# xmindflow/TransCeption

Hardware: AMD Instinct MI355X
Metric: images/sec fwd+bwd at 224x224 B=16 per GPU (higher is better)
Workload: dtype bf16; 1 GPU; TransCeption (MSTransception) 224x224 B=16/GPU fwd+bwd+SGD, synthetic Synapse npz slices via the device loader, name-seeded random-init weights; global_batch=16, image_size=224, parallelism=dp1, headline_mode=loader, headline_degraded=False, launch_mode=hipGraph replay

## Files before the change

transception_amd/_header.py:

```python
from __future__ import annotations

import ctypes as C
import operator
import os
import re
from typing import NamedTuple

HEADER = os.path.join(os.path.dirname(os.path.dirname(os.path.abspath(__file__))), "include", "transception_hip.h")


class SideHeader(NamedTuple):
    attr: str
    file: str
    version: str
    entry: str
    what: str

    @property
    def path(self) -> str:
        return os.path.join(os.path.dirname(HEADER), self.file)


SIDE_HEADERS = (SideHeader("POST", "transception_post.h", "TC_POST_ABI_VERSION", "tc_post_abi_version", "post-processing"),
                SideHeader("EMA", "transception_ema.h", "TC_EMA_ABI_VERSION", "tc_ema_abi_version", "weight-averaging"),
                SideHeader("TTA", "transception_tta.h", "TC_TTA_ABI_VERSION", "tc_tta_abi_version", "test-time augmentation"),
                SideHeader("RESAMPLE", "transception_resample.h", "TC_RESAMPLE_ABI_VERSION", "tc_resample_abi_version", "score resampling"),
                SideHeader("BRIDGE", "transception_bridge.h", "TC_BRIDGE_ABI_VERSION", "tc_bridge_abi_version", "bridge LayerNorm"),
                SideHeader("LOSS", "transception_loss.h", "TC_LOSS_ABI_VERSION", "tc_loss_abi_version", "focal / Tversky loss"))

SCALARS = {"int": C.c_int, "long long": C.c_longlong, "float": C.c_float, "double": C.c_double,
           "unsigned": C.c_uint, "unsigned int": C.c_uint}
POINTEES = set(SCALARS) | {"void", "unsigned char"}


class HeaderError(ValueError):
    pass


class Function(NamedTuple):
    restype: type
    argtypes: list
    query: bool


class Header(NamedTuple):
    functions: dict
    structs: dict
    constants: dict


_TOKEN = re.compile(r"\s*(\d+|<<|[()|+-])")
_LEVELS = ({"|": operator.or_}, {"<<": operator.lshift}, {"+": operator.add, "-": operator.sub})


def evaluate(expr: str) -> int:
    toks, pos, expr = [], 0, expr.strip()
    while pos < len(expr):
        m = _TOKEN.match(expr, pos)
        if not m:
            raise HeaderError(f"constant expression {expr!r}: cannot read {expr[pos:]!r}")
        toks.append(m.group(1))
        pos = m.end()
    toks.reverse()

    def level(i):
        if i == len(_LEVELS):
            t = toks.pop() if toks else ""
            if t in ("-", "+"):
                return level(i) if t == "+" else -level(i)
            if t == "(":
                v = level(0)
                if not toks or toks.pop() != ")":
                    raise HeaderError(f"constant expression {expr!r}: missing )")
                return v
            if t.isdigit():
                return int(t)
            raise HeaderError(f"constant expression {expr!r}: operand expected")
        v = level(i + 1)
        while toks and toks[-1] in _LEVELS[i]:
            v = _LEVELS[i][toks.pop()](v, level(i + 1))
# ... 102 lines not shown
```

transception_amd/_lib.py:

```python
from __future__ import annotations

import ctypes as C
import os

from . import _header

HERE = os.path.dirname(os.path.abspath(__file__))
LIB_PATH = os.environ.get("TC_LIB_PATH") or os.path.join(HERE, "libtransception_hip.so")

ABI = _header.load()
SIGNATURES = {name: f.argtypes for name, f in ABI.functions.items()}
K, S = ABI.constants, ABI.structs
SIDE = {s.attr: _header.load(s.path) for s in _header.SIDE_HEADERS}
POST, EMA, TTA, RESAMPLE, BRIDGE, LOSS = SIDE["POST"], SIDE["EMA"], SIDE["TTA"], SIDE["RESAMPLE"], SIDE["BRIDGE"], SIDE["LOSS"]

ABI_VERSION = K["TC_ABI_VERSION"]
TC_F32, TC_BF16, TC_F16 = K["TC_F32"], K["TC_BF16"], K["TC_F16"]
ACT_NONE, ACT_HSWISH, ACT_COORD, ACT_SIGMOID = K["TC_ACT_NONE"], K["TC_ACT_HSWISH"], K["TC_ACT_COORD"], K["TC_ACT_SIGMOID"]
ACT_GELU, ACT_SCALE, ACT_RELU = K["TC_ACT_GELU"], K["TC_ACT_SCALE"], K["TC_ACT_RELU"]
FFN_NONE, FFN_LN_A, FFN_LN_B, FFN_EP = K["TC_FFN_NONE"], K["TC_FFN_LN_A"], K["TC_FFN_LN_B"], K["TC_FFN_EP"]
EW_PATCHIFY, EW_DEINTERLEAVE, EW_COPY, EW_MULTI_MAX = K["TC_EW_PATCHIFY"], K["TC_EW_DEINTERLEAVE"], K["TC_EW_COPY"], K["TC_EW_MULTI_MAX"]
TC_AUG_WARP, TC_AUG_LINEAR, TC_AUG_BLUR, TC_AUG_PIECEWISE = K["TC_AUG_WARP"], K["TC_AUG_LINEAR"], K["TC_AUG_BLUR"], K["TC_AUG_PIECEWISE"]
TC_AUG_SKIP, TC_AUG_FROM_RAW = K["TC_AUG_SKIP"], K["TC_AUG_FROM_RAW"]
ATTN_DKV_SPLITS = K["TC_ATTN_DKV_SPLITS"]
TC_METRIC_NO_SOURCE, TC_METRIC_SELECT_WORK_BYTES = K["TC_METRIC_NO_SOURCE"], K["TC_METRIC_SELECT_WORK_BYTES"]
TC_IGNORE_NONE = K["TC_IGNORE_NONE"]
POST_ABI_VERSION, EMA_ABI_VERSION, TTA_ABI_VERSION, RESAMPLE_ABI_VERSION, BRIDGE_ABI_VERSION, LOSS_ABI_VERSION = (SIDE[s.attr].constants[s.version] for s in _header.SIDE_HEADERS)
TC_OVERLAP_DICE, TC_OVERLAP_TVERSKY = LOSS.constants["TC_OVERLAP_DICE"], LOSS.constants["TC_OVERLAP_TVERSKY"]
TC_CC_LARGEST, TC_CC_MIN_VOXELS = POST.constants["TC_CC_LARGEST"], POST.constants["TC_CC_MIN_VOXELS"]
TC_RESAMPLE_MAX_EXTENT = RESAMPLE.constants["TC_RESAMPLE_MAX_EXTENT"]
TC_TTA_FLIP_H, TC_TTA_FLIP_W, TC_TTA_TRANSPOSE = TTA.constants["TC_TTA_FLIP_H"], TTA.constants["TC_TTA_FLIP_W"], TTA.constants["TC_TTA_TRANSPOSE"]

TcGemm, TcLnFold, TcDwFold, TcDwSeg, TcFfnSeg = S["TcGemm"], S["TcLnFold"], S["TcDwFold"], S["TcDwSeg"], S["TcFfnSeg"]
TcFfnFused, TcFfnBwd, TcEffAtt, TcEwSeg, TcSliceAug = S["TcFfnFused"], S["TcFfnBwd"], S["TcEffAtt"], S["TcEwSeg"], S["TcSliceAug"]
TcSrSrc, TcLnSeg = BRIDGE.structs["TcSrSrc"], BRIDGE.structs["TcLnSeg"]
SR_LN_MAX, LN_MULTI_MAX = BRIDGE.constants["TC_SR_LN_MAX"], BRIDGE.constants["TC_LN_MULTI_MAX"]


class TcError(RuntimeError):
    pass


class _Lib:
    calls = 0

    def __init__(self, path: str = LIB_PATH):
        if not os.path.exists(path):
            raise TcError(f"{path} is missing: build it with `python -m transception_amd.build` "
                          "(there is no CPU/PyTorch fallback for the TransCeption hot path)")
        self.path = path
        self.cdll = C.CDLL(path)
        headers = [(ABI, "TC_ABI_VERSION", "tc_abi_version", "ABI"),
                   *((SIDE[s.attr], s.version, s.entry, s.what + " ABI") for s in _header.SIDE_HEADERS)]
        for header, *_ in headers:
            for name, f in header.functions.items():
                fn = getattr(self.cdll, name)
                fn.argtypes = f.argtypes
                fn.restype = f.restype
                setattr(self, name, fn if f.query else self._checked(name, fn))
        for header, version, entry, what in headers:
            v, host = getattr(self.cdll, entry)(), header.constants[version]
            if v != host:
                raise TcError(f"{what} mismatch: library {v}, host {host}")

    @staticmethod
    def _checked(name, fn):
        def call(*a):
            _Lib.calls += 1
            rc = fn(*a)
            if rc != 0:
                raise TcError(f"{name} failed with status {rc}")
        call.__name__ = name
        return call


_lib = None


def lib() -> _Lib:
    global _lib
# ... 4 lines not shown
```

transception_amd/csrc/factoratt.hip:

```cpp
#include "tc_common.h"

namespace {

constexpr int FA_MAXCH = 64;

template <typename T>
__device__ __forceinline__ void fa_load_tile(float* dst, const T* src, int ld, int N, int Ch) {
    constexpr int VEC = TcVec16<T>::N;
    const int nv = Ch / VEC, total = N * nv;
#pragma unroll 4
    for (int i = threadIdx.x; i < total; i += 256) {
        const int n = i / nv, cv = i - n * nv;
        const uint4 r = *reinterpret_cast<const uint4*>(src + (long long)n * ld + cv * VEC);
        tc_unpack16<T>(r, dst + n * Ch + cv * VEC);
    }
}

__device__ __forceinline__ void fa_softmax_cols(float* e, float* cmax, float* cinv, float* red, int N, int Ch) {
    const int tid = threadIdx.x, R = 256 / Ch, c = tid % Ch, r = tid / Ch;
    float m = -INFINITY;
    if (r < R) for (int n = r; n < N; n += R) m = fmaxf(m, e[n * Ch + c]);
    if (r < R) red[r * Ch + c] = m;
    __syncthreads();
    if (tid < Ch) { float v = red[tid]; for (int i = 1; i < R; ++i) v = fmaxf(v, red[i * Ch + tid]); cmax[tid] = v; }
    __syncthreads();
    float s = 0.f;
    if (r < R) {
        const float mc = cmax[c];
        for (int n = r; n < N; n += R) { const float v = __expf(e[n * Ch + c] - mc); e[n * Ch + c] = v; s += v; }
        red[r * Ch + c] = s;
    }
    __syncthreads();
    if (tid < Ch) { float v = 0.f; for (int i = 0; i < R; ++i) v += red[i * Ch + tid]; cinv[tid] = 1.0f / v; }
    __syncthreads();
}

template <typename T>
__device__ __forceinline__ void fa_load_tile_raw(T* dst, const T* src, int ld, int N, int Ch) {
    constexpr int VEC = TcVec16<T>::N;
    const int nv = Ch / VEC, total = N * nv;
#pragma unroll 4
    for (int i = threadIdx.x; i < total; i += 256) {
        const int n = i / nv, cv = i - n * nv;
        *reinterpret_cast<uint4*>(dst + n * Ch + cv * VEC) = *reinterpret_cast<const uint4*>(src + (long long)n * ld + cv * VEC);
    }
}
__device__ __forceinline__ float fa_get(const float* p, int i) { return p[i]; }
__device__ __forceinline__ float fa_get(const bf16_t* p, int i) { return bf2f(p[i]); }
__device__ __forceinline__ float fa_get(const f16_t* p, int i) { return h2f(p[i]); }
__device__ __forceinline__ void fa_get8(const float* p, float* o) {
    const float4 a = *reinterpret_cast<const float4*>(p), b = *reinterpret_cast<const float4*>(p + 4);
    o[0] = a.x; o[1] = a.y; o[2] = a.z; o[3] = a.w; o[4] = b.x; o[5] = b.y; o[6] = b.z; o[7] = b.w;
}
// ... 938 lines not shown
            const T* src = xb + (long long)((ok ? yy : y) * p.W + (ok ? xx : x)) * p.ldx + sub * 8;
#pragma unroll
            for (int v = 0; v < NVL; ++v) {
                raw[ky * 3 + kx][v] = *reinterpret_cast<const uint4*>(src + v * 64);
                if (!ok) raw[ky * 3 + kx][v] = make_uint4(0u, 0u, 0u, 0u);
            }
        }
    __syncthreads();
    float t1v[NVL][8];
    float s1 = 0.f;
#pragma unroll
    for (int v = 0; v < NVL; ++v) {
        const int c0 = v * 64 + sub * 8;
        float acc[8], ctr[8];
        tc_unpack16<T>(raw[4][v], ctr);
#pragma unroll
        for (int u = 0; u < 8; ++u) acc[u] = bs[c0 + u];
#pragma unroll
        for (int tap = 0; tap < 9; ++tap) {
            float xv[8], w8[8];
            tc_unpack16<T>(raw[tap][v], xv);
            fa_get8(wt + tap * C + c0, w8);
#pragma unroll
            for (int u = 0; u < 8; ++u) acc[u] = fmaf(xv[u], w8[u], acc[u]);
        }
#pragma unroll
        for (int u = 0; u < 8; ++u) acc[u] += ctr[u];
        const uint4 pk = tc_pack16<T>(acc);
        if (live) *reinterpret_cast<uint4*>(reinterpret_cast<T*>(p.t1) + (grow + r) * p.ldt + c0) = pk;
        tc_unpack16<T>(pk, t1v[v]);
#pragma unroll
        for (int u = 0; u < 8; ++u) s1 += t1v[v][u];
    }
    const float mean = tc_group_sum<8>(s1) * (1.0f / C);
    float s2 = 0.f;
#pragma unroll
    for (int v = 0; v < NVL; ++v)
#pragma unroll
        for (int u = 0; u < 8; ++u) { const float d = t1v[v][u] - mean; s2 += d * d; }
    const float rstd = rsqrtf(tc_group_sum<8>(s2) * (1.0f / C) + p.eps);
    if (live) {
#pragma unroll
        for (int v = 0; v < NVL; ++v) {
            const int c0 = v * 64 + sub * 8;
            float o[8];
#pragma unroll
            for (int u = 0; u < 8; ++u) o[u] = (t1v[v][u] - mean) * rstd * gm[c0 + u] + bt[c0 + u];
            *reinterpret_cast<uint4*>(reinterpret_cast<T*>(p.xn) + (grow + r) * p.ldn + c0) = tc_pack16<T>(o);
        }
        if (sub == 0) { p.mean[grow + r] = mean; p.rstd[grow + r] = rstd; }
    }
}

static size_t mhca_att_smem_of(int C, int N) {
    return C == 64 ? mhca_att_smem<64>(N) : C == 128 ? mhca_att_smem<128>(N) : C == 320 ? mhca_att_smem<320>(N) : 0;
}
extern "C" int tc_mhca_att_supported(int C, int N, int dtype) {
    if (dtype != TC_BF16 && dtype != TC_F16) return 0;
    const size_t sm = mhca_att_smem_of(C, N);
    return sm > 0 && sm <= 150 * 1024 && N > 0;
}
extern "C" int tc_mhca_att_fwd(const void* xn, int ldx, const void* Wqkv, const void* bqkv, const void* w3, const void* b3, const void* w5,
                               const void* b5, const void* w7, const void* b7, long long gs, void* qkv, int ldq, void* convv, int ldc,
                               void* o, int ldo, float* stats, int groups, int B, int H, int W, int C, float scale, int dtype, void* stream) {
    if (!xn || !Wqkv || !bqkv || !w3 || !b3 || !w5 || !b5 || !w7 || !b7 || !qkv || !convv || !o || !stats || groups <= 0 || B <= 0 || H <= 0 || W <= 0)
        return TC_ERR_ARG;
    if (!tc_mhca_att_supported(C, H * W, dtype)) return TC_ERR_UNSUPPORTED;
    {
        const long long n = (long long)H * W, lmax = ldx > ldq ? (ldx > ldc ? ldx : ldc) : (ldq > ldc ? ldq : ldc);
        if (n * (lmax > ldo ? lmax : ldo) >= (1LL << 31) || lmax >= (1 << 23) || ldo >= (1 << 23)) return TC_ERR_ARG;
    }
    if (ldx % 8 || ldq % 8 || ldc % 8 || ldo % 8 || gs % 8 ||
        (((uintptr_t)xn | (uintptr_t)Wqkv | (uintptr_t)qkv | (uintptr_t)convv | (uintptr_t)o) & 15))
        return TC_ERR_ARG;
    MhcaAttDev p;
    p.xn = xn; p.Wqkv = Wqkv; p.bqkv = bqkv; p.cw[0] = w3; p.cw[1] = w5; p.cw[2] = w7; p.cb[0] = b3; p.cb[1] = b5; p.cb[2] = b7;
    p.qkv = qkv; p.convv = convv; p.o = o; p.stats = stats; p.gs = gs; p.ldx = ldx; p.ldq = ldq; p.ldc = ldc; p.ldo = ldo;
    p.B = B; p.N = H * W; p.H = H; p.W = W; p.scale = scale;
    const int Bt = groups * B;
    hipStream_t s = (hipStream_t)stream;
    if (dtype == TC_BF16) {
        if (C == 64) return mhca_att_launch<bf16_t, 64>(p, Bt, s);
        if (C == 128) return mhca_att_launch<bf16_t, 128>(p, Bt, s);
        return mhca_att_launch<bf16_t, 320>(p, Bt, s);
    }
    if (C == 64) return mhca_att_launch<f16_t, 64>(p, Bt, s);
    if (C == 128) return mhca_att_launch<f16_t, 128>(p, Bt, s);
    return mhca_att_launch<f16_t, 320>(p, Bt, s);
}

static size_t mhca_att_bwd_smem_of(int C, int N) {
    return C == 64 ? mhca_att_bwd_smem<64>(N) : C == 128 ? mhca_att_bwd_smem<128>(N) : C == 320 ? mhca_att_bwd_smem<320>(N) : 0;
}
extern "C" int tc_mhca_att_bwd_supported(int C, int N, int dtype) {
    if (dtype != TC_BF16 && dtype != TC_F16) return 0;
    const size_t sm = mhca_att_bwd_smem_of(C, N);
    return sm > 0 && sm <= 79 * 1024 && N > 0;
}
extern "C" int tc_mhca_att_bwd(const void* qkv, int ldq, const void* convv, int ldc, const void* go, int ldgo, const float* stats, void* dqkv,
                               int ldd, int acc_q, int acc_k, int acc_v, const void* w3, const void* w5, const void* w7, float* dw3, float* db3,
                               float* dw5, float* db5, float* dw7, float* db7, long long gs, int groups, int B, int H, int W, int C, float scale,
                               int dtype, void* stream) {
    if (!qkv || !convv || !go || !stats || !dqkv || !w3 || !w5 || !w7 || !dw3 || !db3 || !dw5 || !db5 || !dw7 || !db7 || groups <= 0 || B <= 0 ||
        H <= 0 || W <= 0)
        return TC_ERR_ARG;
    if (!tc_mhca_att_bwd_supported(C, H * W, dtype)) return TC_ERR_UNSUPPORTED;
    {
        const long long n = (long long)H * W, l1 = ldq > ldc ? ldq : ldc, l2 = ldgo > ldd ? ldgo : ldd, lmax = l1 > l2 ? l1 : l2;
        if (n * lmax >= (1LL << 31) || lmax >= (1 << 23)) return TC_ERR_ARG;
    }
    if (ldq % 8 || ldc % 8 || ldgo % 8 || ldd % 8 || (((uintptr_t)qkv | (uintptr_t)convv | (uintptr_t)go | (uintptr_t)dqkv) & 15)) return TC_ERR_ARG;
    MhcaAttBwdDev p;
    p.qkv = qkv; p.convv = convv; p.go = go; p.cw[0] = w3; p.cw[1] = w5; p.cw[2] = w7; p.stats = stats; p.dqkv = dqkv;
    p.dcw[0] = dw3; p.dcw[1] = dw5; p.dcw[2] = dw7; p.dcb[0] = db3; p.dcb[1] = db5; p.dcb[2] = db7; p.gs = gs;
    p.ldq = ldq; p.ldc = ldc; p.ldgo = ldgo; p.ldd = ldd; p.acc_q = acc_q; p.acc_k = acc_k; p.acc_v = acc_v;
    p.B = B; p.N = H * W; p.H = H; p.W = W; p.scale = scale;
    const int Bt = groups * B;
    hipStream_t s = (hipStream_t)stream;
    if (dtype == TC_BF16) {
        if (C == 64) return mhca_att_bwd_launch<bf16_t, 64>(p, Bt, s);
        if (C == 128) return mhca_att_bwd_launch<bf16_t, 128>(p, Bt, s);
        return mhca_att_bwd_launch<bf16_t, 320>(p, Bt, s);
    }
    if (C == 64) return mhca_att_bwd_launch<f16_t, 64>(p, Bt, s);
    if (C == 128) return mhca_att_bwd_launch<f16_t, 128>(p, Bt, s);
    return mhca_att_bwd_launch<f16_t, 320>(p, Bt, s);
}

extern "C" int tc_dw_ln_supported(int C, int dtype) { return (dtype == TC_BF16 || dtype == TC_F16) && (C == 64 || C == 128 || C == 320); }
extern "C" int tc_dw_ln_fwd(const void* x, int ldx, const void* w, const void* b, long long wstride, const void* gamma, const void* beta,
                            long long gstride, void* t1, int ldt, void* xn, int ldn, float* mean, float* rstd, int groups, int B, int H, int W,
                            int C, float eps, int dtype, void* stream) {
    if (!x || !w || !b || !gamma || !beta || !t1 || !xn || !mean || !rstd || groups <= 0 || B <= 0 || H <= 0 || W <= 0) return TC_ERR_ARG;
    if (!tc_dw_ln_supported(C, dtype)) return TC_ERR_UNSUPPORTED;
    if (ldx % 8 || ldt % 8 || ldn % 8 || (((uintptr_t)x | (uintptr_t)t1 | (uintptr_t)xn) & 15)) return TC_ERR_ARG;
    DwLnDev p;
    p.x = x; p.w = w; p.b = b; p.gamma = gamma; p.beta = beta; p.t1 = t1; p.xn = xn; p.mean = mean; p.rstd = rstd;
    p.wstride = wstride; p.gstride = gstride; p.ldx = ldx; p.ldt = ldt; p.ldn = ldn; p.B = B; p.H = H; p.W = W;
    p.rows_per_group = B * H * W; p.eps = eps;
    const dim3 grid((p.rows_per_group + 31) / 32, groups);
    hipStream_t s = (hipStream_t)stream;
#define DWLN(TT, CC) hipLaunchKernelGGL((dw_ln_fwd_kernel<TT, CC>), grid, dim3(256), 0, s, p)
    if (dtype == TC_BF16) { if (C == 64) DWLN(bf16_t, 64); else if (C == 128) DWLN(bf16_t, 128); else DWLN(bf16_t, 320); }
    else { if (C == 64) DWLN(f16_t, 64); else if (C == 128) DWLN(f16_t, 128); else DWLN(f16_t, 320); }
#undef DWLN
    return tc_launch_status();
}
```

transception_amd/engine.py:

```python
from __future__ import annotations

import ctypes as C
import os
from typing import Callable, Dict, List, Optional, Tuple

import torch

from ._lib import (ATTN_DKV_SPLITS, EW_COPY, EW_DEINTERLEAVE, EW_PATCHIFY, TcEffAtt, TcEwSeg, TcFfnBwd, TcFfnFused, ACT_COORD, ACT_GELU, ACT_HSWISH, ACT_NONE, ACT_SCALE, ACT_SIGMOID, FFN_EP, FFN_LN_A, FFN_LN_B, TC_BF16, TC_F16, TC_F32, TcDwFold, TcDwSeg, TcFfnSeg,
                   TcGemm, TcLnFold, TcLnSeg, TcSrSrc, LN_MULTI_MAX, lib)

TC_DTYPE = {torch.float32: TC_F32, torch.bfloat16: TC_BF16, torch.float16: TC_F16}

PROFILE: Optional[dict] = None


SEG_MARKS = os.environ.get("TC_SEG_MARKS", "")
SEG_LABELS: List[str] = []


def _timed(name: str, flops: float, fn):
    if PROFILE is None:
        fn()
        return
    e0, e1 = torch.cuda.Event(enable_timing=True), torch.cuda.Event(enable_timing=True)
# ... 78 lines not shown
    def is_whole(self) -> bool:
        rt = self.root.data
        return self.region == (0, rt.shape[0], 0, rt.shape[1])

    def apply_path(self, t: torch.Tensor) -> torch.Tensor:
        for k in self.path:
            if k[0] == "c":
                t = t[:, k[1]:k[2]]
            elif k[0] == "r":
                t = t[k[1]:k[2]]
            else:
                t = t.view(k[1], k[2])
        return t


def _overlap(a, b) -> bool:
    return a[0] < b[1] and b[0] < a[1] and a[2] < b[3] and b[2] < a[3]


def _ptr(t: Optional[torch.Tensor]):
    return None if t is None else t.data_ptr()


_WORKSPACES: Dict[Tuple[str, str], torch.Tensor] = {}
WORKSPACE_BYTES = 16384 + 1024 * 16384


def _workspace(device, tag: str = "") -> torch.Tensor:
    key = (str(device), tag)
    ws = _WORKSPACES.get(key)
    if ws is None:
        ws = _WORKSPACES[key] = torch.zeros(WORKSPACE_BYTES * (8 if tag == "many" else 1), dtype=torch.uint8, device=device)
    return ws


_SPLITK_CAP = 128
_SPLITK_BLOCKS = 512
_SPLITK_KMIN = 384
_THR128 = 100000
_FFN_STORE_ACT = os.environ.get("TC_FFN_STORE_ACT", "1") != "0"
_FFN_LN_GEMM_MAXC = int(os.environ.get("TC_FFN_LN_GEMM_MAXC", "64"))
_FFN_TILED = os.environ.get("TC_FFN_TILED", "1") != "0"
_DW_DEFER = os.environ.get("TC_DW_DEFER", "1") != "0"
_LN_DEFER = os.environ.get("TC_LN_DEFER", "1") != "0"
_EFFATT_FUSED = os.environ.get("TC_EFFATT_FUSED", "1") != "0"
_FFN_PRE_LN = os.environ.get("TC_FFN_PRE_LN", "0") != "0"
_SR_LN_FUSED = os.environ.get("TC_SR_LN_FUSED", "1") != "0"
_LN_MULTI = os.environ.get("TC_LN_MULTI", "1") != "0"
_PENDING_RES = os.environ.get("TC_PENDING_RES", "1") != "0"
_LIN_LN_FUSED = os.environ.get("TC_LIN_LN_FUSED", "1") != "0"
_RIPM_FUSED = os.environ.get("TC_RIPM_FUSED", "1") != "0"
_LN_CLS_FUSED = os.environ.get("TC_LN_CLS_FUSED", "1") != "0"
_DW_LN_FUSED = os.environ.get("TC_DW_LN_FUSED", "1") != "0"
_MHCA_ATT_BWD_FUSED = os.environ.get("TC_MHCA_ATT_BWD_FUSED", "1") != "0"
_MHCA_ATT_FUSED = os.environ.get("TC_MHCA_ATT_FUSED", "1") != "0"
_DW_BWD_ONE = os.environ.get("TC_DW_BWD_ONE", "1") != "0"
_FFN_TILED_BWD = os.environ.get("TC_FFN_TILED_BWD", "1") != "0"
_FFN_TILE_BWD = (0, 0)
_FFN_TILE = (0, 0)
_POISON = bool(os.environ.get("TC_DEBUG_POISON"))


def _empty(shape, dtype, device) -> torch.Tensor:
    if _POISON:
        return torch.full(tuple(shape), float("nan"), dtype=dtype, device=device)
    return torch.empty(tuple(shape), dtype=dtype, device=device)


_ZERO_NEED: Dict[Tuple[str, torch.dtype], int] = {}


class _ZeroArena:
    def __init__(self, device, dtype):
        self.key = (str(device), dtype)
        self.device, self.dtype = device, dtype
        self.buf: Optional[torch.Tensor] = None
        self.used = 0
        self.asked = 0

    def zeros_like(self, t: torch.Tensor) -> torch.Tensor:
        n = (t.numel() + 127) // 128 * 128
        self.asked += n
        if self.buf is None:
            need = _ZERO_NEED.get(self.key, 0)
            if need >= n:
                self.buf = torch.zeros(need, dtype=self.dtype, device=self.device)
        if self.buf is not None and self.used + n <= self.buf.numel() and t.is_contiguous():
            out = self.buf[self.used:self.used + t.numel()].view(t.shape)
            self.used += n
            return out
        return torch.zeros_like(t)

    def close(self):
        _ZERO_NEED[self.key] = max(self.asked, 0)


class _Grouped:
    def __init__(self, G, n, pgs):
        self.G, self.n, self.pgs, self.prev = G, n, pgs, None

    def __enter__(self):
        self.prev = (self.G.ngroups, self.G.pgs)
        self.G.ngroups, self.G.pgs = self.n, self.pgs
        return self

    def __exit__(self, *a):
# ... 832 lines not shown
        c = x.cols // max(p * p, 1)
        ncls = Wc.data.shape[0]
        rows = B * H * p * W * p if p else x.rows
        out = self.new(rows, (ncls + 7) // 8 * 8).colslice(0, ncls) if pad_rows else self.new(rows, ncls)
        mean, rstd = self.f32(rows), self.f32(rows)
        es = x.data.element_size()
        self.n_launch += 1
        _timed("hbm:ln_cls_fwd (pixel shuffle + LayerNorm + classifier, one launch)", 1.0 * rows * (c + ncls) * es, lambda: self.L.tc_ln_cls_fwd(
            _ptr(x.data), x.ld, _ptr(g.data), _ptr(b.data), _ptr(Wc.data), _ptr(bc.data), _ptr(out.data), out.ld, _ptr(mean), _ptr(rstd),
            B, H, W, p, c, ncls, eps, self.dt, self.stream))

        def bwd():
            dl = self.grad_of(out)
            if dl is None or not x.requires_grad:
                return
            gx, acc = self.wgrad(x)
            assert not acc, "the expanded map has one consumer"
            n = int(self.L.tc_ln_cls_scratch_floats(rows, ncls))
            scratch = self.f32(n)
            _timed("hbm:ln_cls_bwd", 1.0 * rows * (2 * c + ncls) * es, lambda: self.L.tc_ln_cls_bwd(
                _ptr(dl), dl.stride(0), _ptr(x.data), x.ld, _ptr(g.data), _ptr(b.data), _ptr(Wc.data), _ptr(mean), _ptr(rstd), _ptr(gx), gx.stride(0),
                _ptr(g.grad), _ptr(b.grad), _ptr(Wc.grad), _ptr(bc.grad), _ptr(scratch), n, B, H, W, p, c, ncls, self.dt, self.stream))
        self._rec(bwd)
        return out

    def linear_ln_supported(self, x: Var, W: P, residual: Optional[Var], *params: P) -> bool:
        Cc = x.cols
        return (all(q.data.data_ptr() % 16 == 0 for q in params) and _LIN_LN_FUSED and self.dt != TC_F32 and tuple(W.data.shape) == (Cc, Cc) and W.data.is_contiguous()
                and x.ld % 8 == 0 and x.data.data_ptr() % 16 == 0 and (residual is None or (residual.ld % 8 == 0 and residual.data.data_ptr() % 16 == 0))
                and (self.ngroups == 1 or self.pgs % 8 == 0) and bool(self.L.tc_linear_ln_supported(Cc, self.dt)))

    def linear_ln(self, x: Var, W: P, b: P, residual: Optional[Var], g: P, beta: P, eps: float, out: Optional[Var] = None,
                  ln_out: Optional[Var] = None) -> Tuple[Var, Var]:
        Gn = self.ngroups
        t = self.linear(x, W, b, out=out, residual=residual, launch=False)
        mean, rstd = self.f32(x.rows), self.f32(x.rows)
        xn = self.layernorm(t, g, beta, eps, out=ln_out, stats=(mean, rstd), launch=False)
        assert t.rows == x.rows and t.cols == x.cols, "row-stacked groups only"
        self.n_launch += 1
        es = x.data.element_size()
        _timed("hbm:linear_ln_fwd (Linear + residual + LayerNorm, one launch)", (4.0 if residual is not None else 3.0) * x.rows * x.cols * es,
               lambda: self.L.tc_linear_ln_fwd(_ptr(x.data), x.ld, _ptr(W.data), _ptr(b.data), W.gs if Gn > 1 else 0,
                                               _ptr(residual.data) if residual is not None else None, residual.ld if residual is not None else 0,
                                               _ptr(g.data), _ptr(beta.data), g.gs if Gn > 1 else 0, _ptr(t.data), t.ld, _ptr(xn.data), xn.ld,
                                               _ptr(mean), _ptr(rstd), Gn, x.rows // Gn, x.cols, eps, self.dt, self.stream))
        return t, xn

    def dw_ln_supported(self, x: Var) -> bool:
        return (_DW_LN_FUSED and self.dt != TC_F32 and x.ld % 8 == 0 and x.data.data_ptr() % 16 == 0
                and (self.pgs % 8 == 0 or self.ngroups == 1) and bool(self.L.tc_dw_ln_supported(x.cols, self.dt)))

    def dw_ln(self, x: Var, w: P, b: P, g: P, beta: P, B: int, H: int, W: int, eps: float) -> Tuple[Var, Var]:
        Gn = self.ngroups
        t1 = self.dwconv(x, w, b, B, H, W, 3, 1, True, launch=False)
        mean, rstd = self.f32(x.rows), self.f32(x.rows)
        xn = self.layernorm(t1, g, beta, eps, stats=(mean, rstd), launch=False)
        self.n_launch += 1
        es = x.data.element_size()
        _timed("hbm:dw_ln_fwd (cpe dw3x3 + skip + LayerNorm, one launch)", 3.0 * x.rows * x.cols * es, lambda: self.L.tc_dw_ln_fwd(
            _ptr(x.data), x.ld, _ptr(w.data), _ptr(b.data), w.gs if Gn > 1 else 0, _ptr(g.data), _ptr(beta.data), g.gs if Gn > 1 else 0,
            _ptr(t1.data), t1.ld, _ptr(xn.data), xn.ld, _ptr(mean), _ptr(rstd), Gn, B, H, W, x.cols, eps, self.dt, self.stream))
        return t1, xn

    def dwconv(self, x: Var, w: P, b: Optional[P], B: int, H: int, W: int, k: int, stride: int = 1, add_input: bool = False,
               out: Optional[Var] = None, launch: bool = True) -> Var:
        Cc = x.cols
        Gn = self.ngroups
        assert x.rows == Gn * B * H * W and (Gn == 1 or (w.gs > 0 and stride == 1))
        Ho, Wo = (H - 1) // stride + 1, (W - 1) // stride + 1
        if out is None:
            out = self.new(Gn * B * Ho * Wo, Cc)
        es = x.data.element_size()
        if launch:
            _timed("hbm:dwconv_fwd", (x.rows + out.rows) * Cc * es, lambda: self.L.tc_dwconv_fwd(
                _ptr(x.data), x.ld, _ptr(w.data), _ptr(b.data) if b is not None else None, _ptr(out.data), out.ld, B, H, W, Cc, k, stride,
                int(add_input), Gn, w.gs, self.dt, self.stream))

        def bwd():
            dy = self.grad_of(out)
            if dy is None:
                return
            if x.requires_grad and w.grad is not None and stride == 1 and _DW_BWD_ONE:
                gx, acc = self.wgrad(x)
                vec = 16 // es
                db = _ptr(b.grad) if b is not None else None
                tile_ok = not (x.ld % vec or dy.stride(0) % vec or gx.stride(0) % vec or _ptr(dy) % 16 or _ptr(x.data) % 16 or _ptr(gx) % 16)
                self._dw_walkers(
                    (lambda sites, offs: self.L.tc_dwconv_bwd_plan(B, H, W, Cc, k, Gn, self.dt, C.byref(sites[0]))) if _DW_DEFER and tile_ok else None,
                    lambda wsp, wsb: _timed("hbm:dwconv_bwd (input + weight gradient, one launch)", (2.0 * x.rows * (1 + acc) + 2.0 * out.rows) * Cc * es,
                                            lambda: self.L.tc_dwconv_bwd(_ptr(dy), dy.stride(0), _ptr(x.data), x.ld, _ptr(w.data), _ptr(gx), gx.stride(0),
                                                                         _ptr(w.grad), db, B, H, W, Cc, k, int(add_input), acc, Gn, w.gs, wsp, wsb,
                                                                         self.dt, self.stream)),
                    [(_ptr(w.grad), db, None, None, w.gs)])
                return
            if x.requires_grad:
                gx, acc = self.wgrad(x)
                _timed("hbm:dwconv_bwd_input", (x.rows * (1 + acc) + out.rows) * Cc * es, lambda: self.L.tc_dwconv_bwd_input(
                    _ptr(dy), dy.stride(0), _ptr(w.data), _ptr(gx), gx.stride(0), B, H, W, Cc, k, stride, int(add_input), acc, Gn, w.gs,
                    self.dt, self.stream))
            if w.grad is not None:
                ws = _workspace(self.dev)
                _timed("hbm:dwconv_bwd_weight", (x.rows + out.rows) * Cc * es, lambda: self.L.tc_dwconv_bwd_weight(
                    _ptr(dy), dy.stride(0), _ptr(x.data), x.ld, _ptr(w.grad), _ptr(b.grad) if b is not None else None, B, H, W, Cc, k,
                    stride, Gn, w.gs, ws.data_ptr(), ws.numel(), self.dt, self.stream))
        self._rec(bwd)
        return out

    def dwconv_multi(self, xs: List[Var], ws: List[P], bs: List[Optional[P]], geo, ks: List[int], outs: List[Optional[Var]],
                     add_input: bool = False, launch: bool = True) -> List[Var]:
# ... 856 lines not shown
```

Measured before the change: 1518 images/sec.

## Fuse LayerNorm backward with depthwise 3x3 conv backward in one kernel

After: 1516 images/sec. About the same (-0.1%).

```diff
diff --git a/include/transception_mhca.h b/include/transception_mhca.h
--- /dev/null
+++ b/include/transception_mhca.h
@@ -0,0 +1,24 @@
+#ifndef TRANSCEPTION_MHCA_H
+#define TRANSCEPTION_MHCA_H
+
+#ifdef __cplusplus
+extern "C" {
+#endif
+
+#define TC_MHCA_ABI_VERSION 1
+#ifndef TC_QUERY
+#define TC_QUERY
+#endif
+
+TC_QUERY int tc_mhca_abi_version(void);
+
+TC_QUERY int tc_dw_ln_bwd_walkers(int groups, int B, int H, int W, int C, int dtype);
+int tc_dw_ln_bwd(const void* dxn, int lddn, const void* t1, int ldt, const void* x, int ldx, const void* w, long long wstride,
+                 const void* gamma, long long gstride, const float* mean, const float* rstd, const void* dres, int ldres, void* gx, int ldg,
+                 int acc, float* ln_part, long long ln_part_floats, float* dw_part, long long dw_part_floats, int groups, int B, int H, int W,
+                 int C, int dtype, void* stream);
+
+#ifdef __cplusplus
+}
+#endif
+#endif
diff --git a/transception_amd/_header.py b/transception_amd/_header.py
--- a/transception_amd/_header.py
+++ b/transception_amd/_header.py
@@ -26,6 +26,7 @@
                 SideHeader("TTA", "transception_tta.h", "TC_TTA_ABI_VERSION", "tc_tta_abi_version", "test-time augmentation"),
                 SideHeader("RESAMPLE", "transception_resample.h", "TC_RESAMPLE_ABI_VERSION", "tc_resample_abi_version", "score resampling"),
                 SideHeader("BRIDGE", "transception_bridge.h", "TC_BRIDGE_ABI_VERSION", "tc_bridge_abi_version", "bridge LayerNorm"),
+                SideHeader("MHCA", "transception_mhca.h", "TC_MHCA_ABI_VERSION", "tc_mhca_abi_version", "MHCA block backward"),
                 SideHeader("LOSS", "transception_loss.h", "TC_LOSS_ABI_VERSION", "tc_loss_abi_version", "focal / Tversky loss"))
 
 SCALARS = {"int": C.c_int, "long long": C.c_longlong, "float": C.c_float, "double": C.c_double,
diff --git a/transception_amd/_lib.py b/transception_amd/_lib.py
--- a/transception_amd/_lib.py
+++ b/transception_amd/_lib.py
@@ -12,7 +12,7 @@
 SIGNATURES = {name: f.argtypes for name, f in ABI.functions.items()}
 K, S = ABI.constants, ABI.structs
 SIDE = {s.attr: _header.load(s.path) for s in _header.SIDE_HEADERS}
-POST, EMA, TTA, RESAMPLE, BRIDGE, LOSS = SIDE["POST"], SIDE["EMA"], SIDE["TTA"], SIDE["RESAMPLE"], SIDE["BRIDGE"], SIDE["LOSS"]
+POST, EMA, TTA, RESAMPLE, BRIDGE, MHCA, LOSS = (SIDE[s.attr] for s in _header.SIDE_HEADERS)
 
 ABI_VERSION = K["TC_ABI_VERSION"]
 TC_F32, TC_BF16, TC_F16 = K["TC_F32"], K["TC_BF16"], K["TC_F16"]
@@ -25,7 +25,7 @@
 ATTN_DKV_SPLITS = K["TC_ATTN_DKV_SPLITS"]
 TC_METRIC_NO_SOURCE, TC_METRIC_SELECT_WORK_BYTES = K["TC_METRIC_NO_SOURCE"], K["TC_METRIC_SELECT_WORK_BYTES"]
 TC_IGNORE_NONE = K["TC_IGNORE_NONE"]
-POST_ABI_VERSION, EMA_ABI_VERSION, TTA_ABI_VERSION, RESAMPLE_ABI_VERSION, BRIDGE_ABI_VERSION, LOSS_ABI_VERSION = (SIDE[s.attr].constants[s.version] for s in _header.SIDE_HEADERS)
+POST_ABI_VERSION, EMA_ABI_VERSION, TTA_ABI_VERSION, RESAMPLE_ABI_VERSION, BRIDGE_ABI_VERSION, MHCA_ABI_VERSION, LOSS_ABI_VERSION = (SIDE[s.attr].constants[s.version] for s in _header.SIDE_HEADERS)
 TC_OVERLAP_DICE, TC_OVERLAP_TVERSKY = LOSS.constants["TC_OVERLAP_DICE"], LOSS.constants["TC_OVERLAP_TVERSKY"]
 TC_CC_LARGEST, TC_CC_MIN_VOXELS = POST.constants["TC_CC_LARGEST"], POST.constants["TC_CC_MIN_VOXELS"]
 TC_RESAMPLE_MAX_EXTENT = RESAMPLE.constants["TC_RESAMPLE_MAX_EXTENT"]
diff --git a/transception_amd/csrc/factoratt.hip b/transception_amd/csrc/factoratt.hip
--- a/transception_amd/csrc/factoratt.hip
+++ b/transception_amd/csrc/factoratt.hip
@@ -1,4 +1,5 @@
 #include "tc_common.h"
+#include "../../include/transception_mhca.h"
 
 namespace {
 
@@ -1043,6 +1044,256 @@
     }
 }
 
+__device__ __forceinline__ float fa_pin(float v) { asm volatile("" : "+v"(v)); return v; }
+struct DwLnBwdDev {
+    const void *dxn, *t1, *x, *w, *gamma, *dres;
+    void* gx;
+    const float *mean, *rstd;
+    float *ln_part, *dw_part;
+    long long wstride, gstride;
+    int lddn, ldt, ldx, ldres, ldg, acc, B, H, W, tilesW, tilesH;
+};
+template <int C> struct DwLnBwdGeom {
+    static constexpr int CV = C / 8, PIXQ = CV + 1;
+    static constexpr int TS = 8, HS = TS + 2, NH = HS * HS;
+    static constexpr int GS = C == 64 ? 8 : (C == 128 ? 16 : 64), RPB = 256 / GS;
+    static constexpr int CQ = C / 4, PG = 256 / CQ, NPX = (TS * TS + PG - 1) / PG;
+    static constexpr size_t tile_bytes = (size_t)NH * PIXQ * 16, red_bytes = (size_t)RPB * 2 * C * 4, scr_bytes = (size_t)PG * C * 4;
+    static constexpr size_t smem = (tile_bytes > red_bytes ? (tile_bytes > scr_bytes ? tile_bytes : scr_bytes) : (red_bytes > scr_bytes ? red_bytes : scr_bytes)) +
+                                   (size_t)9 * C * 4;
+};
+template <typename T, int C, bool RES>
+__global__ __launch_bounds__(256, 2) void dw_ln_bwd_kernel(DwLnBwdDev p) {
+    using G = DwLnBwdGeom<C>;
+    constexpr int CV = G::CV, PIXQ = G::PIXQ, HS = G::HS, NH = G::NH, GS = G::GS, RPB = G::RPB, PG = G::PG, NPX = G::NPX;
+    constexpr bool V8 = C != 320;
+    constexpr int NV = C / 4;
+    extern __shared__ uint4 dlb_smem[];
+    uint4* gt = dlb_smem;
+    float* wsm = reinterpret_cast<float*>(reinterpret_cast<char*>(dlb_smem) + (G::smem - (size_t)9 * C * 4));
+    const int tid = threadIdx.x, grp = blockIdx.y, bx = blockIdx.x, gxw = gridDim.x;
+    const int gl = tid % GS, gi = tid / GS;
+    const int cq = tid % G::CQ, pg = tid / G::CQ;
+    const bool dwl = pg < PG;
+    typedef unsigned dlb_u2 __attribute__((ext_vector_type(2)));
+    const int hw = p.H * p.W;
+    const long long rows = (long long)p.B * hw, grow = (long long)grp * rows;
+    const T* gamma = reinterpret_cast<const T*>(p.gamma) + grp * p.gstride;
+    {
+        const T* w = reinterpret_cast<const T*>(p.w) + grp * p.wstride;
+        for (int i = tid; i < 9 * C; i += 256) { const int ch = i / 9, tap = i - ch * 9; wsm[(8 - tap) * C + ch] = ldf<T>(w + i); }
+    }
+    const int q0 = V8 ? 2 * gl : gl, q1 = V8 ? 2 * gl + 1 : gl + 64;
+    const bool has1 = q1 < NV;
+    float gm[8], ag[8], ab[8];
+    if constexpr (V8) tc_unpack16<T>(*reinterpret_cast<const uint4*>(gamma + gl * 8), gm);
+    else {
+        const float4 a = ld4<T>(gamma + q0 * 4), b = has1 ? ld4<T>(gamma + q1 * 4) : make_float4(0.f, 0.f, 0.f, 0.f);
+        gm[0] = a.x; gm[1] = a.y; gm[2] = a.z; gm[3] = a.w; gm[4] = b.x; gm[5] = b.y; gm[6] = b.z; gm[7] = b.w;
+    }
+    float wacc[10][4];
+#pragma unroll
+    for (int j = 0; j < 8; ++j) {
+        ag[j] = ab[j] = 0.f;
+#pragma unroll
+        for (int t = 0; t < 10; ++t) wacc[t][j & 3] = 0.f;
+    }
+    constexpr float invC = 1.0f / (float)C;
+    constexpr bool has_res = RES;
+    const T* dxn = reinterpret_cast<const T*>(p.dxn);
+    const T* t1 = reinterpret_cast<const T*>(p.t1);
+    const T* xin = reinterpret_cast<const T*>(p.x);
+    const T* dres = reinterpret_cast<const T*>(p.dres);
+    T* gxo = reinterpret_cast<T*>(p.gx);
+    const int tpi = p.tilesW * p.tilesH, ntiles = p.B * tpi;
+    const SDiv dtpi = sdiv_make(tpi), dtw = sdiv_make(p.tilesW);
+    for (int tile = bx; tile < ntiles; tile += gxw) {
+        const int b = sdiv(tile, dtpi), trem = smod(tile, b, dtpi), ty = sdiv(trem, dtw), tx = smod(trem, ty, dtw);
+        const int oh0 = ty * G::TS, ow0 = tx * G::TS;
+        const long long rowb = grow + (long long)b * hw;
+        auto load_x = [&](int px) {
+            const int oh = oh0 + (px >> 3), ow = ow0 + (px & 7);
+            const bool live = dwl && px < 64 && oh < p.H && ow < p.W;
+            return *reinterpret_cast<const dlb_u2*>(xin + (rowb + (live ? oh * p.W + ow : 0)) * p.ldx + cq * 4);
+        };
+        dlb_u2 xnext = load_x(pg);
+        auto halo_row = [&](int hp, bool& ok, bool& inner) {
+            const int hy = hp / HS, hx = hp - hy * HS, ih = oh0 - 1 + hy, iw = ow0 - 1 + hx;
+            ok = hp < NH && (unsigned)ih < (unsigned)p.H && (unsigned)iw < (unsigned)p.W;
+            inner = ok && hy >= 1 && hy <= G::TS && hx >= 1 && hx <= G::TS;
+            return rowb + (ok ? ih * p.W + iw : 0);
+        };
+        auto ln_row = [&](const int hp, const bool ok, const bool inner, float* xv, float* d, const float* rq, const float mu, const float rs) {
+#pragma unroll
+            for (int j = 0; j < 8; ++j) xv[j] = (xv[j] - mu) * rs;
+            {
+                const float im = inner ? 1.0f : 0.f;
+#pragma unroll
+                for (int j = 0; j < 8; ++j) { const float dm = d[j] * im; ag[j] = fmaf(dm, xv[j], ag[j]); ab[j] += dm; }
+            }
+            float dy[8];
+#pragma unroll
+            for (int j = 0; j < 8; ++j) { dy[j] = d[j]; d[j] = fa_pin(d[j] * gm[j]); }
+            float s1, s2;
+            if constexpr (V8) {
+                s1 = ((d[0] + d[1]) + d[2]) + d[3]; s1 += ((d[4] + d[5]) + d[6]) + d[7];
+                s2 = fmaf(d[3], xv[3], fmaf(d[2], xv[2], fmaf(d[1], xv[1], d[0] * xv[0])));
+                s2 += fmaf(d[7], xv[7], fmaf(d[6], xv[6], fmaf(d[5], xv[5], d[4] * xv[4])));
+            } else {
+                s1 = 0.f + (fmaf(dy[2], gm[2], fmaf(dy[0], gm[0], d[1])) + d[3]);
+                s2 = 0.f + (fmaf(xv[2], d[2], fmaf(xv[1], d[1], xv[0] * d[0])) + fa_pin(xv[3] * d[3]));
+                if (has1) {
+                    s1 += fmaf(dy[6], gm[6], fmaf(dy[4], gm[4], d[5])) + d[7];
+                    s2 += fmaf(xv[6], d[6], fmaf(xv[5], d[5], xv[4] * d[4])) + fa_pin(xv[7] * d[7]);
+                }
+            }
+            s1 = fa_pin(tc_group_sum<GS>(s1) * invC); s2 = fa_pin(tc_group_sum<GS>(s2) * invC);
+            float o[8];
+#pragma unroll
+            for (int j = 0; j < 8; ++j) o[j] = fmaf(-xv[j], s2, d[j] - s1);
+            if constexpr (RES) {
+#pragma unroll
+                for (int j = 0; j < 8; ++j) o[j] = fmaf(rs, o[j], rq[j]);
+            } else {
+#pragma unroll
+                for (int j = 0; j < 8; ++j) o[j] *= rs;
+            }
+            if (hp < NH) {
+                if constexpr (V8) {
+                    gt[hp * PIXQ + gl] = ok ? tc_pack16<T>(o) : make_uint4(0u, 0u, 0u, 0u);
+                } else {
+                    uint2* dst = reinterpret_cast<uint2*>(gt + hp * PIXQ);
+                    dst[q0] = ok ? make_uint2(pack2<T>(o[0], o[1]), pack2<T>(o[2], o[3])) : make_uint2(0u, 0u);
+                    if (has1) dst[q1] = ok ? make_uint2(pack2<T>(o[4], o[5]), pack2<T>(o[6], o[7])) : make_uint2(0u, 0u);
+                }
+            }
+        };
+        if constexpr (V8) {
+            constexpr int UB = 4;
+#pragma unroll 1
+            for (int hp0 = 0; hp0 < NH; hp0 += RPB * UB) {
+                uint4 rx[UB], rd[UB], rr[UB];
+                float mu[UB], rs[UB];
+                bool ok[UB], inner[UB];
+#pragma unroll
+                for (int u = 0; u < UB; ++u) {
+                    const long long row = halo_row(hp0 + u * RPB + gi, ok[u], inner[u]);
+                    rx[u] = *reinterpret_cast<const uint4*>(t1 + row * p.ldt + gl * 8);
+                    rd[u] = *reinterpret_cast<const uint4*>(dxn + row * p.lddn + gl * 8);
+                    rr[u] = make_uint4(0u, 0u, 0u, 0u);
+                    if constexpr (RES) rr[u] = *reinterpret_cast<const uint4*>(dres + row * p.ldres + gl * 8);
+                    mu[u] = p.mean[row]; rs[u] = p.rstd[row];
+                }
+#pragma unroll
+                for (int u = 0; u < UB; ++u) {
+                    float xv[8], d[8], rq[8];
+                    tc_unpack16<T>(rx[u], xv); tc_unpack16<T>(rd[u], d); tc_unpack16<T>(rr[u], rq);
+                    ln_row(hp0 + u * RPB + gi, ok[u], inner[u], xv, d, rq, mu[u], rs[u]);
+                }
+            }
+        } else {
+#pragma unroll 1
+            for (int hp0 = 0; hp0 < NH; hp0 += RPB) {
+                bool ok, inner;
+                const int hp = hp0 + gi;
+                const long long row = halo_row(hp, ok, inner);
+                float xv[8], d[8], rq[8];
+                const int qb = has1 ? q1 : q0;
+                const float4 x0 = ld4<T>(t1 + row * p.ldt + q0 * 4), x1 = ld4<T>(t1 + row * p.ldt + qb * 4);
+                const float4 d0 = ld4<T>(dxn + row * p.lddn + q0 * 4), d1 = ld4<T>(dxn + row * p.lddn + qb * 4);
+                float4 r0 = make_float4(0.f, 0.f, 0.f, 0.f), r1 = r0;
+                if constexpr (RES) { r0 = ld4<T>(dres + row * p.ldres + q0 * 4); r1 = ld4<T>(dres + row * p.ldres + qb * 4); }
+                xv[0] = x0.x; xv[1] = x0.y; xv[2] = x0.z; xv[3] = x0.w; xv[4] = x1.x; xv[5] = x1.y; xv[6] = x1.z; xv[7] = x1.w;
+                d[0] = d0.x; d[1] = d0.y; d[2] = d0.z; d[3] = d0.w; d[4] = d1.x; d[5] = d1.y; d[6] = d1.z; d[7] = d1.w;
+                rq[0] = r0.x; rq[1] = r0.y; rq[2] = r0.z; rq[3] = r0.w; rq[4] = r1.x; rq[5] = r1.y; rq[6] = r1.z; rq[7] = r1.w;
+                ln_row(hp, ok, inner, xv, d, rq, p.mean[row], p.rstd[row]);
+            }
+        }
+        __syncthreads();
+#pragma unroll 1
+        for (int j = 0; j < NPX; ++j) {
+            const int px = pg + j * PG, py = px >> 3, pxx = px & 7, oh = oh0 + py, ow = ow0 + pxx;
+            const dlb_u2 xcur = xnext;
+            if (j + 1 < NPX) xnext = load_x(px + PG);
+            if (!dwl || px >= 64) continue;
+            const bool live = oh < p.H && ow < p.W;
+            float xv[4], a[4], gc[4];
+            unpack2<T>(live ? xcur.x : 0u, xv[0], xv[1]); unpack2<T>(live ? xcur.y : 0u, xv[2], xv[3]);
+#pragma unroll
+            for (int u = 0; u < 4; ++u) a[u] = gc[u] = 0.f;
+#pragma unroll
+            for (int ky = 0; ky < 3; ++ky) {
+#pragma unroll
+                for (int kx = 0; kx < 3; ++kx) {
+                    const int m = ky * 3 + kx;
+                    float gv[4];
+                    const dlb_u2 gr = reinterpret_cast<const dlb_u2*>(gt + ((py + ky) * HS + pxx + kx) * PIXQ)[cq];
+                    unpack2<T>(gr.x, gv[0], gv[1]); unpack2<T>(gr.y, gv[2], gv[3]);
+                    const float4 w4 = *reinterpret_cast<const float4*>(wsm + tc_opaque(m * C + cq * 4));
+                    const float w8[4] = {w4.x, w4.y, w4.z, w4.w};
+#pragma unroll
+                    for (int u = 0; u < 4; ++u) {
+                        a[u] = fmaf(w8[u], gv[u], a[u]);
+                        wacc[8 - m][u] = fmaf(xv[u], gv[u], wacc[8 - m][u]);
+                        if (m == 4) gc[u] = gv[u];
+                    }
+                }
+                if (ky == 1) {
+#pragma unroll
+                    for (int u = 0; u < 4; ++u) a[u] += gc[u];
+                }
+            }
+#pragma unroll
+            for (int u = 0; u < 4; ++u) wacc[9][u] += gc[u];
+            if (live) {
+                T* dst = gxo + (rowb + oh * p.W + ow) * p.ldg + cq * 4;
+                if (p.acc) {
+                    const dlb_u2 old = *reinterpret_cast<const dlb_u2*>(dst);
+                    float q[4];
+                    unpack2<T>(old.x, q[0], q[1]); unpack2<T>(old.y, q[2], q[3]);
+#pragma unroll
+                    for (int u = 0; u < 4; ++u) a[u] += q[u];
+                }
+                dlb_u2 o2;
+                o2.x = pack2<T>(a[0], a[1]); o2.y = pack2<T>(a[2], a[3]);
+                *reinterpret_cast<dlb_u2*>(dst) = o2;
+            }
+        }
+        __syncthreads();
+    }
+    float* red = reinterpret_cast<float*>(dlb_smem);
+    {
+#pragma unroll
+        for (int j = 0; j < 8; ++j) {
+            const int ch = V8 ? gl * 8 + j : (j < 4 ? q0 * 4 + j : q1 * 4 + j - 4);
+            if (j < 4 || V8 || has1) { red[(gi * 2 + 0) * C + ch] = ag[j]; red[(gi * 2 + 1) * C + ch] = ab[j]; }
+        }
+        __syncthreads();
+        float* pp = p.ln_part + ((long long)grp * gxw + bx) * 2 * C;
+        for (int c = tid; c < C; c += 256) {
+            float sa = 0.f, sb = 0.f;
+#pragma unroll
+            for (int w = 0; w < RPB; ++w) { sa += red[(w * 2 + 0) * C + c]; sb += red[(w * 2 + 1) * C + c]; }
+            pp[c] = sa; pp[C + c] = sb;
+        }
+    }
+#pragma unroll
+    for (int t = 0; t < 10; ++t) {
+        __syncthreads();
+        if (dwl) {
+#pragma unroll
+            for (int u = 0; u < 4; ++u) red[pg * C + cq * 4 + u] = wacc[t][u];
+        }
+        __syncthreads();
+        for (int c = tid; c < C; c += 256) {
+            float s = 0.f;
+#pragma unroll
+            for (int w = 0; w < PG; ++w) s += red[w * C + c];
+            p.dw_part[(((long long)grp * (C / 64) + (c >> 6)) * gxw + bx) * 640 + t * 64 + (c & 63)] = s;
+        }
+    }
+}
+
 static size_t mhca_att_smem_of(int C, int N) {
     return C == 64 ? mhca_att_smem<64>(N) : C == 128 ? mhca_att_smem<128>(N) : C == 320 ? mhca_att_smem<320>(N) : 0;
 }
@@ -1137,3 +1388,50 @@
 #undef DWLN
     return tc_launch_status();
 }
+
+extern "C" int tc_mhca_abi_version(void) { return TC_MHCA_ABI_VERSION; }
+
+extern "C" int tc_dw_ln_bwd_walkers(int groups, int B, int H, int W, int C, int dtype) {
+    if (groups <= 0 || B <= 0 || H <= 0 || W <= 0 || !tc_dw_ln_supported(C, dtype)) return 0;
+    const long long tiles = (long long)B * ((H + 7) / 8) * ((W + 7) / 8);
+    if (tiles >= (1LL << 21) || (long long)B * H * W >= (1LL << 31) || groups > 65535) return 0;
+    const long long target = 512 / groups > 0 ? 512 / groups : 1, iters = (tiles + target - 1) / target;
+    return (int)((tiles + iters - 1) / iters);
+}
+
+extern "C" int tc_dw_ln_bwd(const void* dxn, int lddn, const void* t1, int ldt, const void* x, int ldx, const void* w, long long wstride,
+                            const void* gamma, long long gstride, const float* mean, const float* rstd, const void* dres, int ldres, void* gx,
+                            int ldg, int acc, float* ln_part, long long ln_part_floats, float* dw_part, long long dw_part_floats, int groups, int B,
+                            int H, int W, int C, int dtype, void* stream) {
+    if (!dxn || !t1 || !x || !w || !gamma || !mean || !rstd || !gx || !ln_part || !dw_part || groups <= 0 || B <= 0 || H <= 0 || W <= 0) return TC_ERR_ARG;
+    if (!tc_dw_ln_supported(C, dtype)) return TC_ERR_UNSUPPORTED;
+    const int n = tc_dw_ln_bwd_walkers(groups, B, H, W, C, dtype);
+    if (n <= 0 || ln_part_floats < (long long)groups * n * 2 * C || dw_part_floats < (long long)groups * n * 10 * C) return TC_ERR_ARG;
+    if (lddn % 8 || ldt % 8 || ldx % 8 || ldg % 8 || (dres && ldres % 8) || lddn < C || ldt < C || ldx < C || ldg < C || (dres && ldres < C) ||
+        (groups > 1 && (wstride % 8 || gstride % 8)) ||
+        (((uintptr_t)dxn | (uintptr_t)t1 | (uintptr_t)x | (uintptr_t)gx | (uintptr_t)gamma | (uintptr_t)dres) & 15))
+        return TC_ERR_ARG;
+    {
+        const int l1 = lddn > ldt ? lddn : ldt, l2 = ldx > ldg ? ldx : ldg, l3 = l1 > l2 ? l1 : l2, lmax = dres && ldres > l3 ? ldres : l3;
+        if ((long long)H * W * lmax >= (1LL << 31)) return TC_ERR_ARG;
+    }
+    DwLnBwdDev p;
+    p.dxn = dxn; p.t1 = t1; p.x = x; p.w = w; p.gamma = gamma; p.dres = dres; p.gx = gx; p.mean = mean; p.rstd = rstd;
+    p.ln_part = ln_part; p.dw_part = dw_part; p.wstride = wstride; p.gstride = gstride;
+    p.lddn = lddn; p.ldt = ldt; p.ldx = ldx; p.ldres = dres ? ldres : 0; p.ldg = ldg; p.acc = acc; p.B = B; p.H = H; p.W = W;
+    p.tilesW = (W + 7) / 8; p.tilesH = (H + 7) / 8;
+    const dim3 grid(n, groups);
+    hipStream_t s = (hipStream_t)stream;
+#define DWLNB(TT, CC) {                                                                                                                      \
+        constexpr size_t smem = DwLnBwdGeom<CC>::smem;                                                                                      \
+        if (smem > 64 * 1024) {                                                                                                              \
+            (void)hipFuncSetAttribute((const void*)dw_ln_bwd_kernel<TT, CC, true>, hipFuncAttributeMaxDynamicSharedMemorySize, (int)smem);   \
+            (void)hipFuncSetAttribute((const void*)dw_ln_bwd_kernel<TT, CC, false>, hipFuncAttributeMaxDynamicSharedMemorySize, (int)smem);  \
+        }                                                                                                                                   \
+        if (dres) hipLaunchKernelGGL((dw_ln_bwd_kernel<TT, CC, true>), grid, dim3(256), smem, s, p);                                        \
+        else hipLaunchKernelGGL((dw_ln_bwd_kernel<TT, CC, false>), grid, dim3(256), smem, s, p); }
+    if (dtype == TC_BF16) { if (C == 64) DWLNB(bf16_t, 64) else if (C == 128) DWLNB(bf16_t, 128) else DWLNB(bf16_t, 320) }
+    else { if (C == 64) DWLNB(f16_t, 64) else if (C == 128) DWLNB(f16_t, 128) else DWLNB(f16_t, 320) }
+#undef DWLNB
+    return tc_launch_status();
+}
diff --git a/transception_amd/engine.py b/transception_amd/engine.py
--- a/transception_amd/engine.py
+++ b/transception_amd/engine.py
@@ -154,6 +154,8 @@
 _RIPM_FUSED = os.environ.get("TC_RIPM_FUSED", "1") != "0"
 _LN_CLS_FUSED = os.environ.get("TC_LN_CLS_FUSED", "1") != "0"
 _DW_LN_FUSED = os.environ.get("TC_DW_LN_FUSED", "1") != "0"
+_DW_LN_BWD_FUSED = os.environ.get("TC_DW_LN_BWD_FUSED", "1") != "0"
+_DW_LN_BWD_WIDTHS = (64, 128)
 _MHCA_ATT_BWD_FUSED = os.environ.get("TC_MHCA_ATT_BWD_FUSED", "1") != "0"
 _MHCA_ATT_FUSED = os.environ.get("TC_MHCA_ATT_FUSED", "1") != "0"
 _DW_BWD_ONE = os.environ.get("TC_DW_BWD_ONE", "1") != "0"
@@ -1092,9 +1094,44 @@
 
     def dw_ln(self, x: Var, w: P, b: P, g: P, beta: P, B: int, H: int, W: int, eps: float) -> Tuple[Var, Var]:
         Gn = self.ngroups
+        n0 = len(self.tape)
         t1 = self.dwconv(x, w, b, B, H, W, 3, 1, True, launch=False)
         mean, rstd = self.f32(x.rows), self.f32(x.rows)
         xn = self.layernorm(t1, g, beta, eps, stats=(mean, rstd), launch=False)
+        if (self.record and _DW_LN_BWD_FUSED and _LN_DEFER and _DW_DEFER and _DW_BWD_ONE and x.requires_grad and x.cols in _DW_LN_BWD_WIDTHS
+                and all(q.grad is not None for q in (w, b, g, beta)) and len(self.tape) == n0 + 2):
+            bw_ln, bw_dw = self.tape.pop(), self.tape.pop()
+            Cc = x.cols
+
+            def bwd():
+                dy = self.grad_of(xn)
+                if dy is None or dy.stride(0) % 8 or _ptr(dy) % 16:
+                    bw_ln()
+                    bw_dw()
+                    return
+                pend = self._take_pending(t1)
+                if pend:
+                    dres, ldres = pend[0], pend[1]
+                else:
+                    gt = self.grad_of(t1)
+                    dres, ldres = (_ptr(gt), gt.stride(0)) if gt is not None else (None, 0)
+                gx, acc = self.wgrad(x)
+                n = int(self.L.tc_dw_ln_bwd_walkers(Gn, B, H, W, Cc, self.dt))
+                nl, nd = Gn * n * 2 * Cc, Gn * n * 10 * Cc
+                lpart, dpart = self.f32(nl), self.f32(nd)
+                es = x.data.element_size()
+                _timed("hbm:dw_ln_bwd (LayerNorm + cpe dw3x3 backward, one launch)", (4.0 + (dres is not None) + acc) * x.rows * Cc * es,
+                       lambda: self.L.tc_dw_ln_bwd(_ptr(dy), dy.stride(0), _ptr(t1.data), t1.ld, _ptr(x.data), x.ld, _ptr(w.data), w.gs,
+                                                   _ptr(g.data), g.gs, _ptr(mean), _ptr(rstd), dres, ldres, _ptr(gx), gx.stride(0), acc,
+                                                   _ptr(lpart), nl, _ptr(dpart), nd, Gn, B, H, W, Cc, self.dt, self.stream))
+                site = TcDwFold()
+                site.part, site.dw, site.db, site.dgamma, site.dbeta, site.wstride = _ptr(dpart), _ptr(w.grad), _ptr(b.grad), None, None, w.gs
+                site.C, site.k, site.groups, site.ch, site.chunks, site.gx, site.nt = Cc, 3, Gn, 64, Cc // 64, n, 10
+                self._dw_pending.append((site, dpart))
+                self._ln_pending.append((lpart, g.grad, beta.grad, g.gs, n, Cc, Gn))
+                if len(self._ln_pending) == 64:
+                    self._flush_param_folds()
+            self._rec(bwd)
         self.n_launch += 1
         es = x.data.element_size()
         _timed("hbm:dw_ln_fwd (cpe dw3x3 + skip + LayerNorm, one launch)", 3.0 * x.rows * x.cols * es, lambda: self.L.tc_dw_ln_fwd(
```
